# JuliaLinearAlgebra/AlgebraicMultigrid.jl

Measured on AMD Instinct MI355X. Metric: V-cycle unknowns/sec + fine-level SpMV GB/s (% HBM peak), 3-D Poisson 256^3, higher is better.
Workload: dtype f64

## Files before the change

### algebraicmultigrid.jl_amd/csrc/hip/amghip.hip

```cpp
#include "amghip_internal.hpp"
#include "gs_schedule.hpp"
#include "csr_ops.hpp"
#include "gmres_kernels.hpp"

namespace {

constexpr int64_t kGraphAutoRows = 65536;

struct Level {
  int64_t n = 0, nc = 0;
  amgh_csr A, S, P, R;
  bool has_S = false;
  amgh_smoother_t pre{}, post{};
  real *res = nullptr, *cx = nullptr, *cb = nullptr, *tmp = nullptr;
  real* il = nullptr;
  amgh_csr* smat() { return has_S ? &S : &A; }
  amgh_csr Pp, Rp;
  bool lo_ok = false;
  real* lo_val = nullptr;
  CodedCols lo_cc;
  bool r_stream = false, p_stream = false;
  bool lo_want = false;
  bool coarse_lo = false;
  bool nat_freed = false;
// ... 1323 lines not shown
}

static int ensure_pcg_bufs(amgh_t* h) {
  if (h->pc_r) return AMGH_OK;
  const int64_t n = fine_n(h);
  RC_TRY(dev_alloc(&h->pc_r, n));
  RC_TRY(dev_alloc(&h->pc_c, n));
  RC_TRY(dev_alloc(&h->pc_u, n));
  h->ws_bytes += 3 * kRealB * n;
  return AMGH_OK;
}

int amgh_solve_d(amgh_t* h, const real* b_d, real* x_d, int cycle_, int maxiter, double abstol, double reltol,
                 int calculate_residual, real* resid_hist, int* iters) {
  RC_TRY(check_ready(h));
  if (!b_d || !x_d || cycle_ < 0 || cycle_ > 2 || maxiter < 0) return AMGH_EINVAL;
  HIP_TRY(hipSetDevice(h->device));
  return solve_dev(h, b_d, x_d, cycle_, maxiter, abstol, reltol, calculate_residual, resid_hist, iters);
}

int amgh_solve(amgh_t* h, const real* b, real* x, int cycle_, int maxiter, double abstol, double reltol,
               int calculate_residual, real* resid_hist, int* iters) {
  RC_TRY(check_ready(h));
  if (!b || !x || cycle_ < 0 || cycle_ > 2 || maxiter < 0) return AMGH_EINVAL;
  HIP_TRY(hipSetDevice(h->device));
  const int64_t n = fine_n(h) * h->nrhs;
  HIP_TRY(hipMemcpyAsync(h->b0, b, sizeof(real) * n, hipMemcpyHostToDevice, h->stream));
  HIP_TRY(hipMemcpyAsync(h->x0, x, sizeof(real) * n, hipMemcpyHostToDevice, h->stream));
  RC_TRY(solve_dev(h, h->b0, h->x0, cycle_, maxiter, abstol, reltol, calculate_residual, resid_hist, iters));
  HIP_TRY(hipMemcpy(x, h->x0, sizeof(real) * n, hipMemcpyDeviceToHost));
  return AMGH_OK;
}

int amgh_precond_apply_d(amgh_t* h, const real* r_d, real* z_d, int cycle_) {
  RC_TRY(check_ready(h));
  if (!r_d || !z_d || cycle_ < 0 || cycle_ > 2) return AMGH_EINVAL;
  HIP_TRY(hipSetDevice(h->device));
  RC_TRY(bw_err_check());
  RC_TRY(vec_fill(h, z_d, fine_n(h) * h->nrhs, 0.0));
  return apply_cycle(h, z_d, r_d, cycle_, true);
}

int amgh_precond_apply(amgh_t* h, const real* r, real* z, int cycle_) {
  RC_TRY(check_ready(h));
  if (!r || !z) return AMGH_EINVAL;
  HIP_TRY(hipSetDevice(h->device));
  const int64_t n = fine_n(h) * h->nrhs;
  HIP_TRY(hipMemcpyAsync(h->b0, r, sizeof(real) * n, hipMemcpyHostToDevice, h->stream));
  RC_TRY(amgh_precond_apply_d(h, h->b0, h->x0, cycle_));
  HIP_TRY(hipStreamSynchronize(h->stream));
  RC_TRY(prof_flush(h));
  RC_TRY(bw_err_check());
  HIP_TRY(hipMemcpy(z, h->x0, sizeof(real) * n, hipMemcpyDeviceToHost));
  return AMGH_OK;
}

int amgh_cycle_d(amgh_t* h, int level, real* x_d, const real* b_d, int cycle_) {
  RC_TRY(check_ready(h));
  if (!x_d || !b_d || cycle_ < 0 || cycle_ > 2 || level < 0 || level > (int)h->levels.size()) return AMGH_EINVAL;
  HIP_TRY(hipSetDevice(h->device));
  if (level == (int)h->levels.size()) return coarse_solve(h, x_d, b_d);
  return cycle(h, level, x_d, b_d, cycle_, false);
}

int amgh_set_stream(amgh_t* h, void* stream) {
  if (!h) return AMGH_EINVAL;
  h->ext_stream = true;
  h->own_stream = h->own_stream ? h->own_stream : h->stream;
  h->stream = (hipStream_t)stream;
  return AMGH_OK;
}

// ... 654 lines not shown
  else if (!strcmp(name, "gs_nnz_per_wg")) g_gs_nnz_per_wg = value;
  else if (!strcmp(name, "gs_threads")) g_gs_threads = value;
  else if (!strcmp(name, "gs_block_inverse")) g_gs_block_inverse = value;
  else if (!strcmp(name, "gs_slots")) g_gs_slots = value;
  else if (!strcmp(name, "gs_xcd_map")) g_gs_xcd_map = value;
  else if (!strcmp(name, "gs_lpr")) g_gs_lpr = value;
  else if (!strcmp(name, "gs_il")) g_gs_il = value;
  else if (!strcmp(name, "trim_coded")) g_trim_coded = value;
  else if (!strcmp(name, "gs_wave_quad")) g_gs_wave_quad = value;
  else if (!strcmp(name, "pcg_fused")) g_pcg_fused = value;
  else if (!strcmp(name, "gs_tri_rb")) g_gs_tri_rb = value;
  else if (!strcmp(name, "gs_tri_rb1")) g_gs_tri_rb1 = value;
  else if (!strcmp(name, "gs_dti_pre")) g_gs_dti_pre = value;
  else if (!strcmp(name, "stream_xcd")) g_stream_xcd = value;
  else if (!strcmp(name, "tail_dense_rows")) g_tail_dense_rows = value < 0 ? 0 : value;
  else if (!strcmp(name, "tail_dense")) { g_tail_dense = value; g_sched_epoch++; }
  else if (!strcmp(name, "tail_dense_batch")) g_tail_dense_batch = value;
  else if (!strcmp(name, "gs_lean")) g_gs_lean = value;
  else if (!strcmp(name, "gs_sell")) g_gs_sell = value;
  else if (!strcmp(name, "gs_sample")) g_gs_sample = value;
  else if (!strcmp(name, "gs_tiny")) g_gs_tiny = value;
  else if (!strcmp(name, "gs_bw")) g_gs_bw = value;
  else if (!strcmp(name, "gs_bw_rows")) g_gs_bw_rows = value;
  else if (!strcmp(name, "gs_bw_chain")) g_gs_bw_chain = value;
  else if (!strcmp(name, "gs_bw_flow")) g_gs_bw_flow = value;
  else if (!strcmp(name, "gs_bw_spin")) g_gs_bw_spin = value;
  else if (!strcmp(name, "gs_bw_nc")) g_gs_bw_nc = value;
  else if (!strcmp(name, "gs_bw_nrhs")) g_gs_bw_nrhs = value;
  else if (!strcmp(name, "gs_bw_skip_pub")) g_gs_bw_skip_pub = value;
  else if (!strcmp(name, "gs_bw_min_rows")) g_gs_bw_min_rows = value;
  else if (!strcmp(name, "gs_bw_two_min_rows")) g_gs_bw_two_min_rows = value;
  else if (!strcmp(name, "gs_dup_launch")) g_gs_dup_launch = value < 0 ? 0 : value > 16 ? 16 : value;
  else if (!strcmp(name, "gs_flow_xzero")) g_gs_flow_xzero = value;
  else if (!strcmp(name, "gs_bw_grid")) g_gs_bw_grid = value < 0 ? 0 : value;
  else if (!strcmp(name, "gs_bw_grid_long")) g_gs_bw_grid_long = value < 0 ? 0 : value;
  else if (!strcmp(name, "gs_bw_dict")) g_gs_bw_dict = value != 0;
  else if (!strcmp(name, "gs_bw_inorder")) g_gs_bw_inorder = value != 0;
  else if (!strcmp(name, "stream_code")) g_stream_code = value != 0;
  else if (!strcmp(name, "gs_bw_relay")) g_gs_bw_relay = value == 0 ? 0 : BW_RELAY_W;
  else if (!strcmp(name, "rhs_il")) g_rhs_il = value;
  else if (!strcmp(name, "jacobi_zero")) g_jacobi_zero = value;
  else if (!strcmp(name, "gs_ept")) g_gs_ept = value;
  else if (!strcmp(name, "gs_merge")) g_gs_merge = value;
  else if (!strcmp(name, "gs_merge_force")) g_gs_merge_force = value;
  else if (!strcmp(name, "gs_merge_force_maxn")) g_gs_merge_force_maxn = value;
  else if (!strcmp(name, "gs_zone")) g_gs_zone = value;
  else if (!strcmp(name, "gs_coarse_lo")) g_gs_coarse_lo = value;
  else if (!strcmp(name, "gs_dense_tri")) g_gs_dense_tri = value;
  else if (!strcmp(name, "gs_dense_blk")) g_gs_dense_blk = value;
  else if (!strcmp(name, "gs_zone_t0_ns")) g_gs_zone_t0_ns = value;
  else if (!strcmp(name, "gs_zone_floor_ns")) g_gs_zone_floor_ns = value;
  else if (!strcmp(name, "gs_bigslot")) g_gs_bigslot = value;
  else if (!strcmp(name, "gs_flip")) g_gs_flip = value;
  else if (!strcmp(name, "gs_keep_lo")) g_gs_keep_lo = value;
  else if (!strcmp(name, "gs_super")) g_gs_super = value;
  else if (!strcmp(name, "gs_block_pipe")) g_gs_block_pipe = value;
  else return AMGH_EINVAL;
  ++g_sched_epoch;
  return AMGH_OK;
}

int amgh_debug_chain_timing(int enable, unsigned long long* out8) {
  if (enable && !g_chain_tim) {
    HIP_TRY(hipMalloc((void**)&g_chain_tim, 8 * sizeof(unsigned long long)));
    HIP_TRY(hipMemset(g_chain_tim, 0, 8 * sizeof(unsigned long long)));
  }
// ... 37 lines not shown
```

### algebraicmultigrid.jl_amd/csrc/hip/amghip_internal.hpp

```cpp
#pragma once
#include "amghip_kernels.hpp"
#include "gs_blocks.hpp"
#include "gs_flow.hpp"

#include <algorithm>
#include <chrono>
#include <cmath>
#include <cstdio>
#include <cstring>
#include <atomic>
#include <mutex>
#include <string>
#include <system_error>
#include <thread>
#include <utility>
#include <vector>

#include "../../../include/amghip.h"

using namespace amgh;

#define HIP_TRY(expr)                                   \
  do {                                                  \
    hipError_t e_ = (expr);                             \
// ... 323 lines not shown
int g_gs_block_pipe = 1;
int g_gs_super = 8;
int g_gs_coarse_lo = 1;
int g_gs_keep_lo = 1;
int g_gs_flip = 1;
int g_gs_bigslot = 1;
int g_gs_merge = 16;
int g_gs_zone_t0_ns = 3000;
int g_gs_zone_floor_ns = 0;
int g_gs_zone = 1;
int g_gs_merge_force_maxn = 0;
int g_gs_merge_force = 0;
int g_gs_xcd_map = 1;
int g_gs_slots = 1;
int g_jacobi_zero = 1;
int g_rhs_il = 1;
int g_gs_tiny = 1;
int g_gs_wave_quad = 1;
int g_gs_bw = 1;
int g_gs_bw_rows = 512;
int g_gs_bw_flow = 1;
int g_gs_bw_spin = 0;
int g_gs_bw_skip_pub = -1;
int g_gs_bw_nc = -1;
int g_gs_bw_nrhs = 1;
int g_gs_bw_chain = 1;
int g_stream_code = 1;
int g_trim_coded = 1;
int g_gs_bw_inorder = 0;
int g_gs_bw_dict = 1;
int g_gs_bw_relay = 3;
int g_gs_bw_grid = 0;
int g_gs_bw_grid_long = 512;
int g_gs_flow_xzero = 1;
int g_gs_dup_launch = 0;
int g_gs_bw_two_min_rows = 200000;
int g_gs_bw_min_rows = 30000;
int g_gs_sample = 1;
int g_gs_sell = 1;
int g_gs_lean = -1;
int g_gs_ept = 0;
int g_gs_lpr = 0;
int g_gs_il = 1;
int g_pcg_fused = 1;
int g_tail_dense_rows = 6144;
int g_tail_dense = 1;
int g_tail_dense_batch = 64;
int g_stream_xcd = 1;
int g_gs_dti_pre = 8;
int g_gs_tri_rb1 = 0;
int g_gs_tri_rb = 1;
int g_gs_dense_blk = 4096;
int g_gs_dense_tri = 1;
int g_gs_block_inverse = 1;

std::atomic<unsigned long long> g_sched_epoch{0};

unsigned long long* g_chain_tim = nullptr;

constexpr int kChainWidth = 1024;

__global__ void find_diag_kernel(const int32_t* rowptr, const int32_t* col, const real* val, int n,
                                 int32_t* dpos, real* diag) {
  const int i = blockIdx.x * blockDim.x + threadIdx.x;
  if (i >= n) return;
  int dp = -1;
// ... 54 lines not shown
```

### algebraicmultigrid.jl_amd/csrc/hip/csr_ops.hpp

```cpp
#pragma once
#include <atomic>

namespace {


template <int MODE, class CFG = DefaultCfg, bool CODED = false>
int launch_stream(const StreamArgs& a0, hipStream_t st, int ncolv = 1) {
  const int nrows = a0.row_end - a0.row_begin;
  if (nrows <= 0) return AMGH_OK;
  StreamArgs a = a0;
  a.ncolv = ncolv;
  const int nb = (nrows + CFG::ROWS - 1) / CFG::ROWS;
  const int64_t grid = (CFG::XCD || ncolv > 1) ? (int64_t)((nb + kNumXcd - 1) / kNumXcd) * kNumXcd * ncolv : nb;
  hipLaunchKernelGGL((csr_stream_kernel<MODE, CFG, CODED>), dim3((unsigned)grid), dim3(CFG::THREADS), 0, st, a);
  HIP_TRY(hipGetLastError());
  return AMGH_OK;
}

template <int MODE>
int launch_gs_level(const StreamArgs& a, int rows, hipStream_t st, int ncolv = 1) {
  const int width = a.row_end - a.row_begin;
  const int avg16 = std::max(16, rows);
  rows = 256;
  while (rows > g_gs_min_rows && (int64_t)rows * avg16 > (int64_t)g_gs_nnz_per_wg * 16) rows >>= 1;
// ... 547 lines not shown
  if (g_gs_merge > 1 && !sor && (backward ? g->mb : g->mf)) {
    lay = backward ? g->mb : g->mf;
    tri = backward ? &g->tri_b : &g->tri_f;
    s_key = 1.0;
    both_dirs = g->mf && g->mb;
  } else if (g_gs_merge > 1 && sor) {
    GsSchedule::SorSet* ss = sor_children(g, omega);
    if (ss && (ss->f || ss->b) && g->xstride == g->ncols && first && !x_resident) {
      HIP_TRY(hipStreamSynchronize(st));
      RC_TRY(gs_grow_xp_for_merged(g, &op->bytes));
    }
    if (ss && (backward ? ss->b : ss->f) && g->xstride > g->ncols) {
      lay = backward ? ss->b : ss->f;
      tri = backward ? &ss->tb : &ss->tf;
      s_key = omega;
      flip_scale = 2.0 - omega;
      both_dirs = ss->f && ss->b;
      sor = false;
    }
  }
  const int64_t xs = g->xstride;
  const bool il = g_gs_il && g_gs_lpr != 1 && lay != g && !g->bw.on && (ncolv == 8 || ncolv == 4 || ncolv == 2);
  if (first || !il) g->xil_cols = 0;
  bool il_s_ok = false;
  if (il && g->xil_cap < xs * ncolv) {
    HIP_TRY(hipStreamSynchronize(st));
    ++g_sched_epoch;
    hipFree(g->xil); g->xil = nullptr; g->xil_cap = 0;
    RC_TRY(dev_alloc(&g->xil, xs * ncolv));
    g->xil_cap = xs * ncolv;
    g->bytes += (int64_t)sizeof(real) * xs * ncolv; op->bytes += (int64_t)sizeof(real) * xs * ncolv;
    g->xil_cols = 0;
  }
  if (first) {
    if (!(reuse_b && g->bp_cols == ncolv))
      hipLaunchKernelGGL(gather_perm_kernel, dim3(grid_for(g->n), ncolv), dim3(256), 0, st, b, g->perm, g->bp, (int)g->n,
                         (int64_t)g->n, (int64_t)g->n);
    g->bp_cols = ncolv;
    if (x_resident) {
    } else if (xzero) {
      const bool flow_zero = g_gs_flow_xzero && g->bw.on && g->bw.flow.on && (g_gs_bw_flow || !g->bw.rec) && g->ncols == g->n && lay == g;
      if (!flow_zero) {
        const int64_t cnt = xs * ncolv;
        hipLaunchKernelGGL(fill_kernel, dim3(grid_for(cnt)), dim3(256), 0, st, g->xp, cnt, 0.0);
        if (il) {
          const int64_t ci = g->ncols * ncolv;
          hipLaunchKernelGGL(fill_kernel, dim3(grid_for(ci)), dim3(256), 0, st, g->xil, ci, 0.0);
          g->xil_cols = ncolv;
        }
      }
    } else {
      hipLaunchKernelGGL(gather_perm_kernel, dim3(grid_for(g->ncols), ncolv), dim3(256), 0, st, (const real*)x, g->permx,
                         g->xp, (int)g->ncols, (int64_t)g->ncols, xs);
    }
    HIP_TRY(hipGetLastError());
  }
  real* xp = g->xp;
  const real* rhs = g->bp;
  int64_t ldb = g->n;
  if (first) g->s_dir = -1;
  if (lay != g) {
    const bool flip = g->ncols == g->n && g->diag_nonzero && both_dirs && g_gs_flip &&
                      g->s_dir == (backward ? 0 : 1) && g->s_key == s_key;
    if (flip) {
      if (il) {
        real* sil = g->xil + g->ncols * ncolv;
#define AMGH_FLIP_IL(BS_) hipLaunchKernelGGL((gs_flip_rhs_il_kernel<BS_>), dim3(grid_for(g->n)), dim3(256), 0, st, (const real*)g->bp, \
                         (const real*)lay->diag, (const real*)xp, xp + g->ncols, (int)g->n, (int64_t)g->n, xs, flip_scale, sil)
// ... 30 lines not shown
      ra.row_begin = 0; ra.row_end = (int32_t)g->n;
      ra.ldx = xs; ra.ldy = xs; ra.ldb = g->n;
      RC_TRY(launch_stream<M_RESID>(ra, st, ncolv));
    }
    g->s_dir = backward ? 1 : 0;
    g->s_key = s_key;
    rhs = xp + g->ncols;
    ldb = xs;
  } else {
    g->s_dir = -1;
  }
  if (op->pipe_epoch && !(g->bw.on && g->bw.flow.on && (g_gs_bw_flow || !g->bw.rec))) return AMGH_ESTATE;
  if (g->bw.on) {
    hipError_t e = hipSuccess;
    const bool flow = g->bw.flow.on && (g_gs_bw_flow || !g->bw.rec);
    if (flow) {
      bw::FlowArgs<real> fa{g->bw.blocks, g->bw.flow.fd, g->bw.flow.srec, g->bw.flow.aux, g->bw.ext_col, g->bw.flow.fl_mb, g->bw.flow.fl_slot,
                            g->bw.flow.mbox, rhs, xp, omega, g->bw.head + 1, g->bw.nblocks, (int32_t)g->bw.flow.nmail,
                            g->bw.err, nullptr, (unsigned)g_gs_bw_spin, (int32_t)g_gs_bw_skip_pub};
      fa.ldb = ldb; fa.ldx = xs; fa.mail_stride = g->bw.flow.mail_stride;
      fa.xzero = (g_gs_flow_xzero && first && xzero && !x_resident && g->ncols == g->n) ? 1 : 0;
      if (ncolv > g->bw.flow.mcols) return AMGH_ESTATE;
      const bool dict = g->bw.flow.dict_on && (g_gs_bw_dict || !g->bw.flow.srec);
      if (op->pipe_epoch) {
        if (ncolv != 1 || !g->bw.flow.xon) return AMGH_ESTATE;
        fa.aux = g->bw.flow.xaux; fa.fl_mb = g->bw.flow.xfl_mb; fa.fl_slot = g->bw.flow.xfl_slot; fa.xlist = g->bw.flow.xlist;
        fa.epoch = op->pipe_epoch; fa.rmbox = op->pipe_rmbox; fa.grid = op->pipe_grid;
        if (dict) { fa.crec = g->bw.flow.crec; fa.dict = g->bw.flow.dict; fa.dict_ent = g->bw.flow.dict_ent; }
        e = bw::sweep_relay<real>(fa, g->bw.maxk, dict ? g->bw.flow.dict_lds : g->bw.flow.lds_max, sor, backward, st, BW_RELAY_W);
      } else if (ncolv == 1 && g_gs_bw_relay > 0) {
        fa.grid = g->bw.maxk > 6 ? (dict ? 0 : g_gs_bw_grid_long) : g_gs_bw_grid;
        fa.late = (g->bw.flow.late_ok && !g_gs_bw_inorder) ? 1 : 0;
        if (dict) { fa.crec = g->bw.flow.crec; fa.dict = g->bw.flow.dict; fa.dict_ent = g->bw.flow.dict_ent; }
        e = bw::sweep_relay<real>(fa, g->bw.maxk, dict ? g->bw.flow.dict_lds : g->bw.flow.lds_max, sor, backward, st, BW_RELAY_W);
      } else {
        if (dict) {
          fa.crec = g->bw.flow.crec; fa.dict = g->bw.flow.dict; fa.dict_ent = g->bw.flow.dict_ent;
          fa.dict_lds = (int32_t)(g->bw.flow.dict_lds - g->bw.flow.lds_max);
        }
        e = bw::sweep_flow<real>(fa, g->bw.maxk, g->bw.flow.lds_max, sor, backward, st, ncolv, g_gs_bw_nc >= 0 ? g_gs_bw_nc : (fa.crec ? 3 : 2));
      }
    } else {
      bw::Args<real> ba{g->bw.blocks, g->bw.rec, g->bw.ext_col, rhs, xp, ldb, xs, omega, 0, nullptr};
      if (g_gs_bw_chain && ncolv == 1 && g->bw.flags) {
        bw::ChainArgs<real> ca{ba, backward ? g->bw.sdep_ptr : g->bw.dep_ptr, backward ? g->bw.sdep : g->bw.dep, g->bw.flags, g->bw.head,
                               g->bw.nblocks, g->bw.err};
        e = bw::sweep_chain<real>(ca, g->bw.maxk, g->bw.lds_max, sor, backward, st);
      } else {
        e = bw::sweep<real>(ba, g->bw.maxk, g->bw.launch_ptr, g->bw.lds_max, sor, backward, ncolv, st);
      }
    }
    if (e != hipSuccess) return -(1000 + (int)e);
  }
  if (il) {
    if (g->xil_cols != ncolv) RC_TRY(il_copy_rows(ncolv, xp, xs, g->xil, 0, il_s_ok ? g->ncols : xs, st));
    else if (!il_s_ok) RC_TRY(il_copy_rows(ncolv, xp, xs, g->xil, g->ncols, g->n, st));
    g->xil_cols = ncolv;
  }
  const int ns = (int)lay->segs.size();
  for (int kk = 0; kk < ns * (1 + g_gs_dup_launch); ++kk) {
    const int k = kk / (1 + g_gs_dup_launch);
    const GsSchedule::Seg& s = lay->segs[backward ? ns - 1 - k : k];
    if (s.chain) {
      ChainArgs c{};
      c.col = lay->col; c.val = lay->val; c.x = xp; c.bp = rhs; c.diag = lay->diag;
      c.rowmeta = lay->rowmeta; c.desc = lay->desc; c.omega = omega; c.tim = g_chain_tim;
// ... 61 lines not shown
        SlotIlArgs ia{};
        ia.wcol = sa.wcol; ia.wval = sa.wval; ia.slot_row = sa.slot_row; ia.wmeta = sa.wmeta; ia.diag = sa.diag;
        ia.xil = g->xil; ia.x = xp; ia.omega = omega; ia.slot0 = s.slot0; ia.nslots = s.nslots;
        ia.xcd_map = (g_gs_xcd_map && s.nslots >= 768) ? 1 : 0;
        ia.soff = (int32_t)g->ncols; ia.ldx = xs;
        const int grid = ia.xcd_map ? ((s.nslots + kNumXcd - 1) / kNumXcd) * kNumXcd : s.nslots;
        RC_TRY(launch_slot_il(ia, sor, ncolv, grid, st));
        HIP_TRY(hipGetLastError());
        continue;
      }
      const int ncv = (ncolv % 8 == 0) ? 8 : (ncolv % 4 == 0) ? 4 : (ncolv % 2 == 0) ? 2 : 1;
      sa.ncolv = ncolv / ncv;
      const int grid = ((xmap || sa.ncolv > 1) ? ((s.nslots + kNumXcd - 1) / kNumXcd) * kNumXcd : s.nslots) * sa.ncolv;
      int lpr = 1;
      if (lay != g && ncolv == 1 && g_gs_lpr != 1) {
        const int avg = s.rows / 16;
        lpr = g_gs_lpr > 1 ? g_gs_lpr : (avg >= 56 ? 16 : avg >= 48 ? 8 : 1);
      }
      int ept = 1;
      if (lay != g && ncolv == 1) ept = g_gs_ept > 0 ? g_gs_ept : ((s.nslots > 1024 && lpr == 1 && s.rows / 16 < 16) ? 2 : 1);
      if (lpr > 1 || ept > 1) { RC_TRY(launch_slot_lpr(sa, sor, lpr, ept, grid, st)); HIP_TRY(hipGetLastError()); continue; }
      RC_TRY(launch_slot(sa, sor, ncv, grid, st));
      HIP_TRY(hipGetLastError());
    } else {
      StreamArgs a{};
      a.rowptr = lay->rowptr; a.col = lay->col; a.val = lay->val;
      a.x = xp; a.y = xp; a.b = rhs; a.dpos = lay->dpos; a.diag = lay->diag; a.perm = nullptr; a.omega = omega;
      a.row_begin = lay->lvl_ptr[s.l0]; a.row_end = lay->lvl_ptr[s.l0 + 1];
      a.ldx = xs; a.ldy = xs; a.ldb = ldb;
      RC_TRY(sor ? launch_gs_level<M_SOR>(a, s.rows, st, ncolv) : launch_gs_level<M_GS>(a, s.rows, st, ncolv));
      if (il) RC_TRY(il_copy_rows(ncolv, xp, xs, g->xil, a.row_begin, a.row_end - a.row_begin, st));
    }
  }
  if (last && !no_scatter) {
    hipLaunchKernelGGL(scatter_perm_kernel, dim3(grid_for(g->n), ncolv), dim3(256), 0, st, (const real*)xp, g->perm, x,
                       (int)g->n, xs, (int64_t)g->n);
    HIP_TRY(hipGetLastError());
  }
  return AMGH_OK;
}

}
```

### algebraicmultigrid.jl_amd/csrc/hip/gs_flow.hpp

```cpp
#pragma once
#include "gs_blocks.hpp"

namespace amgh {
namespace bw {

constexpr int32_t kPubFwd = 1 << 30;
constexpr int32_t kPubBwd = (int32_t)(1u << 31);
constexpr int32_t kPubMask = (1 << 30) - 1;
#ifndef BW_FLOW_WAVES
#define BW_FLOW_WAVES 4
#endif
#ifndef BW_FLOW_DEPTH
#define BW_FLOW_DEPTH 4
#endif

struct FlowDesc {
  int32_t aux;
  int32_t npost;
  int32_t pad0, pad1;
};
constexpr int kStepRowBits = 11, kStepCntBits = 7, kStepNeedMax = (1 << 14) - 1;
inline uint32_t step_word(int r0, int nr, int need) { return (uint32_t)r0 | ((uint32_t)nr << kStepRowBits) | ((uint32_t)need << (kStepRowBits + kStepCntBits)); }

constexpr int32_t kRemoteCell = (int32_t)(1u << 31);
// ... 341 lines not shown
    }
  }
  return true;
}

typedef unsigned int u32x4 __attribute__((ext_vector_type(4)));
typedef unsigned int u32x2 __attribute__((ext_vector_type(2)));

template <typename R>
struct FlowArgs {
  const Desc* blocks; const FlowDesc* fd;
  const unsigned char* srec; const uint32_t* aux;
  const int32_t* ext_col; const int32_t* fl_mb; const uint16_t* fl_slot;
  void* mbox;
  const R* b; R* x; R omega;
  unsigned long long* head;
  int32_t nblocks;
  int32_t nmail;
  int32_t* err;
  long long* tim;
  unsigned int spin_limit;
  int32_t skip_pub;
  int64_t ldb = 0, ldx = 0, mail_stride = 0;
  int32_t lds_stride = 0;
  int32_t ncols = 1, ngroups = 1;
  int32_t xzero = 0;
  uint32_t epoch = 0;
  const unsigned char* crec = nullptr; const unsigned char* dict = nullptr; const int32_t* dict_ent = nullptr;
  int32_t dict_lds = 0;
  const int32_t* xlist = nullptr;
  const void* rmbox = nullptr;
  int32_t late = 0;
  int32_t grid = 0;
};

template <typename R> struct Mail;
template <> struct Mail<double> {
  static constexpr int kBytes = 16;
  typedef u32x4 cell;
  static __device__ __forceinline__ cell load(__amdgpu_buffer_rsrc_t rs, unsigned off) { return __builtin_amdgcn_raw_buffer_load_b128(rs, off, 0, 16); }
  static __device__ __forceinline__ cell load_sys(__amdgpu_buffer_rsrc_t rs, unsigned off) { return __builtin_amdgcn_raw_buffer_load_b128(rs, off, 0, 17); }
  static __device__ __forceinline__ void store(__amdgpu_buffer_rsrc_t rs, unsigned off, double v, unsigned epoch) {
    const unsigned long long u = (unsigned long long)__double_as_longlong(v);
    cell c; c.x = (unsigned)u; c.y = epoch; c.z = (unsigned)(u >> 32); c.w = epoch;
    __builtin_amdgcn_raw_buffer_store_b128(c, rs, off, 0, 16);
  }
  static __device__ __forceinline__ bool valid(const cell& c, unsigned epoch) { return c.y == epoch && c.w == epoch; }
  static __device__ __forceinline__ double value(const cell& c) { return __longlong_as_double((long long)(((unsigned long long)c.z << 32) | c.x)); }
};
template <> struct Mail<float> {
  static constexpr int kBytes = 8;
  typedef u32x2 cell;
  static __device__ __forceinline__ cell load(__amdgpu_buffer_rsrc_t rs, unsigned off) { return __builtin_amdgcn_raw_buffer_load_b64(rs, off, 0, 16); }
  static __device__ __forceinline__ cell load_sys(__amdgpu_buffer_rsrc_t rs, unsigned off) { return __builtin_amdgcn_raw_buffer_load_b64(rs, off, 0, 17); }
  static __device__ __forceinline__ void store(__amdgpu_buffer_rsrc_t rs, unsigned off, float v, unsigned epoch) {
    cell c; c.x = __float_as_uint(v); c.y = epoch;
    __builtin_amdgcn_raw_buffer_store_b64(c, rs, off, 0, 16);
  }
  static __device__ __forceinline__ bool valid(const cell& c, unsigned epoch) { return c.y == epoch; }
  static __device__ __forceinline__ float value(const cell& c) { return __uint_as_float(c.x); }
};

typedef unsigned int u32x3 __attribute__((ext_vector_type(3)));
typedef int i32x4 __attribute__((ext_vector_type(4)));
template <int NDW> struct Dw;
template <> struct Dw<1> { typedef unsigned int type; };
// ... 515 lines not shown
```

### algebraicmultigrid.jl_amd/csrc/hip/gs_relay.hpp

```cpp
#pragma once
#include "gs_flow.hpp"

namespace amgh {
namespace bw {

#ifndef BW_RELAY_W
#define BW_RELAY_W 3
#endif

#ifndef BW_RELAY_SPIN
#define BW_RELAY_SPIN 48u
#endif
#ifndef BW_RELAY_DEPTH_SHORT
#define BW_RELAY_DEPTH_SHORT 3
#endif
#ifndef BW_RELAY_DEPTH_LONG
#define BW_RELAY_DEPTH_LONG 2
#endif
template <int MAXK> struct RelayDepth { static constexpr int value = MAXK <= 12 ? BW_RELAY_DEPTH_SHORT : BW_RELAY_DEPTH_LONG; };
#ifndef BW_RELAY_FETCH_SLEEP
#define BW_RELAY_FETCH_SLEEP 4
#endif
#ifndef BW_RELAY_FETCH_PD
#define BW_RELAY_FETCH_PD 1
// ... 28 lines not shown
  const int ns = d.nlev;
  const int nxb = (int)(((size_t)(d.nrows + d.next + 1) * sizeof(R) + 15) & ~(size_t)15);
  const unsigned spin_limit = a.spin_limit ? a.spin_limit : (1u << 22);
  unsigned char* lds = lds_all;
  R* xl = (R*)lds;
  unsigned int* ctl = (unsigned int*)(lds + nxb);
  R* x = a.x;
  if (fetcher) {
    constexpr int EU = 4;
    const R* xc = uniform_ptr(x);
    const int nfar = BWD ? d.npre + (d.next - d.npre - f.npost) : d.next - d.npre;
    if (a.xzero) {
      for (int e0 = 0; e0 < d.next; e0 += 64) { const int i = e0 + lane; if (i < d.next) xl[d.nrows + i] = (R)0; }
    } else
    for (int e0 = 0; e0 < nfar; e0 += 64 * EU) {
      int32_t ec[EU]; int es[EU];
#pragma unroll
      for (int k = 0; k < EU; ++k) {
        const int i = e0 + lane + 64 * k;
        es[k] = BWD ? (i < d.npre ? i : i + f.npost) : d.npre + i;
        ec[k] = a.ext_col[i < nfar ? d.ext0 + es[k] : 0];
      }
#pragma unroll
      for (int k = 0; k < EU; ++k) pin(ec[k]);
      R xe[EU];
#pragma unroll
      for (int k = 0; k < EU; ++k) xe[k] = xc[ec[k]];
#pragma unroll
      for (int k = 0; k < EU; ++k) pin(xe[k]);
#pragma unroll
      for (int k = 0; k < EU; ++k) { const int i = e0 + lane + 64 * k; if (i < nfar) xl[d.nrows + es[k]] = xe[k]; }
    }
    if (lane == 0) { xl[d.nrows + d.next] = (R)0; ctl[0] = 0u; ctl[1] = 0u; ctl[2] = 0u; ctl[3] = 0u; }
    fetcher_barrier();
#ifdef BW_RELAY_FETCH_PRIO
    __builtin_amdgcn_s_setprio(BW_RELAY_FETCH_PRIO);
#endif
    constexpr int U = 3;
    int nf = BWD ? f.npost : d.npre;
    int f0 = d.ext0 + (BWD ? d.npre : 0);
    if (a.xlist) {
      const int l0 = a.xlist[4 * (int64_t)ob], lf = a.xlist[4 * (int64_t)ob + 1], lb = a.xlist[4 * (int64_t)ob + 2];
      nf = __builtin_amdgcn_readfirstlane(BWD ? lb : lf);
      f0 = __builtin_amdgcn_readfirstlane(BWD ? l0 + lf : l0);
    }
    const __amdgpu_buffer_rsrc_t rs_mail = __builtin_amdgcn_make_buffer_rsrc(uniform_ptr(a.mbox), 0, 0x7ffffff0, 0x00020000);
    const __amdgpu_buffer_rsrc_t rs_rmail = __builtin_amdgcn_make_buffer_rsrc(uniform_ptr(const_cast<void*>(a.rmbox ? a.rmbox : (const void*)a.mbox)), 0, 0x7ffffff0, 0x00020000);
    unsigned total_spins = 0;
    bool fail = false;
#ifdef BW_RELAY_STAMPS
    long long* t_seen = a.tim + 4 * (int64_t)a.nblocks + 384 * (int64_t)a.nblocks + ((int64_t)a.nmail + 1024);
    long long poll_sum = 0, poll_max = 0, npoll = 0;
#endif
#if BW_RELAY_FETCH_PD > 1 && !defined(BW_RELAY_STAMPS)
    constexpr int PD = BW_RELAY_FETCH_PD;
    for (int w0 = 0; w0 < nf && !fail; w0 += 64 * U) {
      int32_t mb[U]; int slot[U]; bool ok[U];
#pragma unroll
      for (int u = 0; u < U; ++u) {
        const int e = w0 + 64 * u + lane;
        mb[u] = a.fl_mb[e < nf ? f0 + e : f0];
        slot[u] = a.fl_slot[e < nf ? f0 + e : f0];
        ok[u] = !(e < nf);
      }
      int first = 0;
      typename M::cell q[PD][U];
// ... 125 lines not shown
      asm_load<O::CTAIL + 1>(o.ct, voff, rs_rec, s0 + (unsigned)(O::NCC - 1) * sd);
    } else {
#pragma unroll
      for (int c = 0; c < O::NVC - 1; ++c) asm_load<4>(o.vf[c], voff, rs_rec, s0 + (unsigned)c * sd);
      asm_load<O::VTAIL>(o.vt, voff, rs_rec, s0 + (unsigned)(O::NVC - 1) * sd);
#pragma unroll
      for (int c = 0; c < O::NCC - 1; ++c) asm_load<4>(o.cf[c], voff, rs_rec, s0 + (unsigned)(O::NVC + c) * sd);
      asm_load<O::CTAIL + 1>(o.ct, voff, rs_rec, s0 + (unsigned)(O::NVC + O::NCC - 1) * sd);
    }
    asm_load<RB / 4>(o.bb, (unsigned)tt * RB, rs_b, (unsigned)r0 * RB);
  };
  O ops[D];
  {
    constexpr int XW = W >= 4 ? 2 : 4;
    if (a.xzero) {
      for (int p = wv * 64 + lane; p < d.nrows; p += 64 * W) xl[p] = (R)0;
    } else
    for (int p0 = wv * 64 * XW; p0 < d.nrows; p0 += 64 * XW * W) {
      R xv[XW];
#pragma unroll
      for (int k = 0; k < XW; ++k) { const int p = p0 + lane + 64 * k; xv[k] = x[d.row0 + (p < d.nrows ? p : 0)]; }
#pragma unroll
      for (int k = 0; k < XW; ++k) pin(xv[k]);
#pragma unroll
      for (int k = 0; k < XW; ++k) { const int p = p0 + lane + 64 * k; if (p < d.nrows) xl[p] = xv[k]; }
    }
    if constexpr (DICT) {
      const int32_t de = a.dict_ent[ob];
      const int nchunk = (((unsigned)de >> 24) + 1) * NVC;
      const u32x4* dg = (const u32x4*)(a.dict + (size_t)(de & 0xffffff) * 16);
      u32x4* dl = (u32x4*)(lds + nxb + 16);
      for (int i = wv * 64 + lane; i < nchunk; i += 64 * W) dl[i] = dg[i];
    }
    asm volatile("s_waitcnt vmcnt(0)" ::: "memory");
#pragma unroll
    for (int j = 0; j < D; ++j) issue(ops[j], wv + j * W);
  }
  __syncthreads();
  __builtin_amdgcn_s_setprio(2);
  const long long t_loaded = a.tim ? wall_clock64() : 0;
  const int32_t pubdir = BWD ? kPubBwd : kPubFwd;
  const bool mute = a.skip_pub == tk;
  const unsigned spare = (unsigned)a.nmail + (unsigned)(ob & 1023);
  bool gave_up = false, bail = false;
  const unsigned xl_base = (unsigned)__builtin_amdgcn_readfirstlane((int)lds_addr(xl));
  const unsigned ctl_off = xl_base + (unsigned)nxb;
  const unsigned dict_base = ctl_off + 16u;
#ifdef BW_RELAY_STAMPS
  const unsigned stamp_base = xl_base + (unsigned)nxb + 16u;
  i32x4 rs_pub = make_rsrc(a.tim + 4 * (int64_t)a.nblocks + 384 * (int64_t)a.nblocks);
  if (!a.tim) rs_pub.z = 0;
#endif
  auto step = [&](const O& o, int kk) {
#ifdef BW_RELAY_STAMPS
    const long long t_rec = wall_clock64();
#endif
    constexpr bool PRE = MAXK <= 18;
    constexpr int NOFF = (PRE && !LATE) ? MAXK : 1;
    auto col_addr = [&](int k) {
      const u32x4 cw = o.cchunk(k >> 3);
      const unsigned w = ((k >> 1) & 3) == 0 ? cw.x : ((k >> 1) & 3) == 1 ? cw.y : ((k >> 1) & 3) == 2 ? cw.z : cw.w;
      return xl_base + ((k & 1) ? (w >> 16) : (w & 0xffffu));
    };
    unsigned off[NOFF];
#pragma unroll
    for (int k = 0; k < NOFF; ++k) off[k] = col_addr(k);
    const int32_t pw = o.pub();
// ... 176 lines not shown
#endif
  };
#ifdef BW_RELAY_STAMPS
  constexpr int L = O::NLOAD, S = 3;
#else
  constexpr int L = O::NLOAD, S = 2;
#endif
  const int nsw = ns > wv ? (ns - wv + W - 1) / W : 0;
  int k = 0;
  if (nsw >= D) {
#pragma unroll
    for (int j = 0; j < D; ++j) {
      if (j == 0) flow_wait<(D - 1) * L>(ops[0]);
      else if (j == 1) flow_wait<(D - 2) * L + 1 * (L + S)>(ops[1 < D ? 1 : 0]);
      else if (j == 2) flow_wait<(D > 2 ? D - 3 : 0) * L + 2 * (L + S)>(ops[2 < D ? 2 : 0]);
      else flow_wait<(D > 3 ? D - 4 : 0) * L + 3 * (L + S)>(ops[3 < D ? 3 : 0]);
      step(ops[j], wv + j * W);
      issue(ops[j], wv + (j + D) * W);
    }
    for (k = D; k + D <= nsw; k += D) {
#pragma unroll
      for (int j = 0; j < D; ++j) {
        flow_wait<(D - 1) * (L + S)>(ops[j]);
        step(ops[j], wv + (k + j) * W);
        issue(ops[j], wv + (k + j + D) * W);
      }
    }
  }
  asm volatile("s_waitcnt vmcnt(0)" ::: "memory");
#pragma unroll
  for (int j = 0; j < D - 1; ++j)
    if (k + j < nsw) { flow_wait<0>(ops[j]); step(ops[j], wv + (k + j) * W); }
  if (gave_up && lane == 0) *a.err = 2;
#ifdef BW_RELAY_STAMPS
  if (a.tim) {
    asm volatile("s_waitcnt lgkmcnt(0)" ::: "memory");
    for (int kk = wv; kk < ns && kk < 128; kk += W)
      if (lane < 3) a.tim[4 * (int64_t)a.nblocks + 384 * (int64_t)ob + 3 * kk + lane] = lds_get<long long>(stamp_base + 24u * (unsigned)kk + 8u * (unsigned)lane);
  }
#endif
  if (a.tim && lane == 0) {
    long long* tt = a.tim + 4 * (int64_t)ob;
    if (wv == 0) {
      tt[0] = t_start; tt[1] = t_loaded;
      unsigned xcc = 0;
#ifdef BW_RELAY_STAMPS
      asm volatile("s_getreg_b32 %0, hwreg(HW_REG_XCC_ID)" : "=s"(xcc));
#endif
      tt[3] = (long long)(xcc & 15u);
    }
    if (wv == (ns - 1) % W) tt[2] = wall_clock64();
  }
}

template <typename R, bool SOR, bool BWD, int MAXK, int W, bool DICT = false, bool LATE = false>
__global__ __launch_bounds__(64 * (W + 1), DICT ? RelayWavesD<MAXK>::value : RelayWaves<MAXK>::value) void gs_bw_relay_kernel(FlowArgs<R> a) {
  extern __shared__ __attribute__((aligned(16))) unsigned char lds_all[];
  static_assert(W >= 2 && W <= 7, "walker waves per block");
  const int wv = __builtin_amdgcn_readfirstlane((int)(threadIdx.x >> 6));
  const int lane = (int)(threadIdx.x & 63u);
  const unsigned int units = (unsigned int)a.nblocks;
  const bool persistent = gridDim.x < units;
  const unsigned int draws = units + (persistent ? gridDim.x : 0u);
  unsigned long long* s_ticket = (unsigned long long*)lds_all;
  if (blockIdx.x < 2048u) for (unsigned i = 0; i < (blockIdx.x >> 5); ++i) __builtin_amdgcn_s_sleep(14);
  for (;;) {
// ... 107 lines not shown
```

Baseline: 1.191 billion.

## Fold permutation gather/scatter into relay GS sweep and skip fine x zero-fill

```diff
diff --git a/algebraicmultigrid.jl_amd/csrc/hip/amghip.hip b/algebraicmultigrid.jl_amd/csrc/hip/amghip.hip
--- a/algebraicmultigrid.jl_amd/csrc/hip/amghip.hip
+++ b/algebraicmultigrid.jl_amd/csrc/hip/amghip.hip
@@ -1379,12 +1379,21 @@
   return AMGH_OK;
 }
 
+bool fine_x_write_only(const amgh_t* h, int cyc) {
+  if (!g_gs_bw_fold || h->levels.empty() || tail_here(h, 0, cyc)) return false;
+  Level* L = h->levels[0];
+  const GsSchedule* g = L->smat()->gs;
+  const bool lo = L->lo_ok && (g_gs_keep_lo || L->nat_freed) && g && g->nblk == 0;
+  auto gs = [](const amgh_smoother_t& s) { return (s.kind == AMGH_SMOOTH_GS || s.kind == AMGH_SMOOTH_SOR) && s.iter > 0; };
+  return lo && g->n == L->n && !(g->dti_f && g_gs_dense_tri && g_gs_block_inverse) && gs(L->pre) && gs(L->post);
+}
+
 int amgh_precond_apply_d(amgh_t* h, const real* r_d, real* z_d, int cycle_) {
   RC_TRY(check_ready(h));
   if (!r_d || !z_d || cycle_ < 0 || cycle_ > 2) return AMGH_EINVAL;
   HIP_TRY(hipSetDevice(h->device));
   RC_TRY(bw_err_check());
-  RC_TRY(vec_fill(h, z_d, fine_n(h) * h->nrhs, 0.0));
+  if (!fine_x_write_only(h, cycle_)) RC_TRY(vec_fill(h, z_d, fine_n(h) * h->nrhs, 0.0));
   return apply_cycle(h, z_d, r_d, cycle_, true);
 }
 
@@ -2105,6 +2114,7 @@
   else if (!strcmp(name, "gs_bw_two_min_rows")) g_gs_bw_two_min_rows = value;
   else if (!strcmp(name, "gs_dup_launch")) g_gs_dup_launch = value < 0 ? 0 : value > 16 ? 16 : value;
   else if (!strcmp(name, "gs_flow_xzero")) g_gs_flow_xzero = value;
+  else if (!strcmp(name, "gs_bw_fold")) g_gs_bw_fold = value != 0;
   else if (!strcmp(name, "gs_bw_grid")) g_gs_bw_grid = value < 0 ? 0 : value;
   else if (!strcmp(name, "gs_bw_grid_long")) g_gs_bw_grid_long = value < 0 ? 0 : value;
   else if (!strcmp(name, "gs_bw_dict")) g_gs_bw_dict = value != 0;
diff --git a/algebraicmultigrid.jl_amd/csrc/hip/amghip_internal.hpp b/algebraicmultigrid.jl_amd/csrc/hip/amghip_internal.hpp
--- a/algebraicmultigrid.jl_amd/csrc/hip/amghip_internal.hpp
+++ b/algebraicmultigrid.jl_amd/csrc/hip/amghip_internal.hpp
@@ -379,6 +379,7 @@
 int g_gs_bw_relay = 3;
 int g_gs_bw_grid = 0;
 int g_gs_bw_grid_long = 512;
+int g_gs_bw_fold = 1;
 int g_gs_flow_xzero = 1;
 int g_gs_dup_launch = 0;
 int g_gs_bw_two_min_rows = 200000;
diff --git a/algebraicmultigrid.jl_amd/csrc/hip/csr_ops.hpp b/algebraicmultigrid.jl_amd/csrc/hip/csr_ops.hpp
--- a/algebraicmultigrid.jl_amd/csrc/hip/csr_ops.hpp
+++ b/algebraicmultigrid.jl_amd/csrc/hip/csr_ops.hpp
@@ -603,8 +603,12 @@
     g->bytes += (int64_t)sizeof(real) * xs * ncolv; op->bytes += (int64_t)sizeof(real) * xs * ncolv;
     g->xil_cols = 0;
   }
+  const bool relay1 = g_gs_bw_fold && ncolv == 1 && g->bw.on && g->bw.flow.on && (g_gs_bw_flow || !g->bw.rec) && g_gs_bw_relay > 0 &&
+                      !op->pipe_epoch && lay == g && g->bw.flow.dict_on && (g_gs_bw_dict || !g->bw.flow.srec);
+  const bool fold_b = relay1 && first && !(reuse_b && g->bp_cols == ncolv);
+  const bool fold_x = relay1 && last && !no_scatter;
   if (first) {
-    if (!(reuse_b && g->bp_cols == ncolv))
+    if (!(reuse_b && g->bp_cols == ncolv) && !fold_b)
       hipLaunchKernelGGL(gather_perm_kernel, dim3(grid_for(g->n), ncolv), dim3(256), 0, st, b, g->perm, g->bp, (int)g->n,
                          (int64_t)g->n, (int64_t)g->n);
     g->bp_cols = ncolv;
@@ -701,6 +705,9 @@
         fa.grid = g->bw.maxk > 6 ? (dict ? 0 : g_gs_bw_grid_long) : g_gs_bw_grid;
         fa.late = (g->bw.flow.late_ok && !g_gs_bw_inorder) ? 1 : 0;
         if (dict) { fa.crec = g->bw.flow.crec; fa.dict = g->bw.flow.dict; fa.dict_ent = g->bw.flow.dict_ent; }
+        if (fold_b || fold_x) fa.perm = g->perm;
+        if (fold_b) fa.b_nat = b;
+        if (fold_x) fa.x_nat = x;
         e = bw::sweep_relay<real>(fa, g->bw.maxk, dict ? g->bw.flow.dict_lds : g->bw.flow.lds_max, sor, backward, st, BW_RELAY_W);
       } else {
         if (dict) {
@@ -828,7 +835,7 @@
       if (il) RC_TRY(il_copy_rows(ncolv, xp, xs, g->xil, a.row_begin, a.row_end - a.row_begin, st));
     }
   }
-  if (last && !no_scatter) {
+  if (last && !no_scatter && !fold_x) {
     hipLaunchKernelGGL(scatter_perm_kernel, dim3(grid_for(g->n), ncolv), dim3(256), 0, st, (const real*)xp, g->perm, x,
                        (int)g->n, xs, (int64_t)g->n);
     HIP_TRY(hipGetLastError());
diff --git a/algebraicmultigrid.jl_amd/csrc/hip/gs_flow.hpp b/algebraicmultigrid.jl_amd/csrc/hip/gs_flow.hpp
--- a/algebraicmultigrid.jl_amd/csrc/hip/gs_flow.hpp
+++ b/algebraicmultigrid.jl_amd/csrc/hip/gs_flow.hpp
@@ -397,6 +397,7 @@
   const void* rmbox = nullptr;
   int32_t late = 0;
   int32_t grid = 0;
+  const int32_t* perm = nullptr; const R* b_nat = nullptr; R* x_nat = nullptr;
 };
 
 template <typename R> struct Mail;
diff --git a/algebraicmultigrid.jl_amd/csrc/hip/gs_relay.hpp b/algebraicmultigrid.jl_amd/csrc/hip/gs_relay.hpp
--- a/algebraicmultigrid.jl_amd/csrc/hip/gs_relay.hpp
+++ b/algebraicmultigrid.jl_amd/csrc/hip/gs_relay.hpp
@@ -84,6 +84,7 @@
       for (int k = 0; k < EU; ++k) { const int i = e0 + lane + 64 * k; if (i < nfar) xl[d.nrows + es[k]] = xe[k]; }
     }
     if (lane == 0) { xl[d.nrows + d.next] = (R)0; ctl[0] = 0u; ctl[1] = 0u; ctl[2] = 0u; ctl[3] = 0u; }
+    if constexpr (DICT) if (a.b_nat) __syncthreads();
     fetcher_barrier();
 #ifdef BW_RELAY_FETCH_PRIO
     __builtin_amdgcn_s_setprio(BW_RELAY_FETCH_PRIO);
@@ -275,7 +276,26 @@
       u32x4* dl = (u32x4*)(lds + nxb + 16);
       for (int i = wv * 64 + lane; i < nchunk; i += 64 * W) dl[i] = dg[i];
     }
+    if (DICT && a.b_nat) {
+      R* bo = const_cast<R*>(a.b) + d.row0;
+      const int32_t* pm = a.perm + d.row0;
+      for (int p0 = wv * 64 * XW; p0 < d.nrows; p0 += 64 * XW * W) {
+        int32_t pi[XW];
+#pragma unroll
+        for (int k = 0; k < XW; ++k) { const int p = p0 + lane + 64 * k; pi[k] = pm[p < d.nrows ? p : 0]; }
+#pragma unroll
+        for (int k = 0; k < XW; ++k) pin(pi[k]);
+        R bv[XW];
+#pragma unroll
+        for (int k = 0; k < XW; ++k) bv[k] = a.b_nat[pi[k]];
+#pragma unroll
+        for (int k = 0; k < XW; ++k) pin(bv[k]);
+#pragma unroll
+        for (int k = 0; k < XW; ++k) { const int p = p0 + lane + 64 * k; if (p < d.nrows) bo[p] = bv[k]; }
+      }
+    }
     asm volatile("s_waitcnt vmcnt(0)" ::: "memory");
+    if constexpr (DICT) if (a.b_nat) __syncthreads();
 #pragma unroll
     for (int j = 0; j < D; ++j) issue(ops[j], wv + j * W);
   }
@@ -518,6 +538,27 @@
   for (int j = 0; j < D - 1; ++j)
     if (k + j < nsw) { flow_wait<0>(ops[j]); step(ops[j], wv + (k + j) * W); }
   if (gave_up && lane == 0) *a.err = 2;
+  if (DICT && a.x_nat) {
+    const unsigned* ctlw = (const unsigned*)(lds + nxb);
+    for (;;) {
+      const unsigned bl = __hip_atomic_load(ctlw + 2, __ATOMIC_RELAXED, __HIP_MEMORY_SCOPE_WORKGROUP);
+      const unsigned dn = __hip_atomic_load(ctlw + 1, __ATOMIC_ACQUIRE, __HIP_MEMORY_SCOPE_WORKGROUP);
+      if (bl != 0u) { bail = true; break; }
+      if (dn >= (unsigned)ns) break;
+      __builtin_amdgcn_s_sleep(1);
+    }
+    if (!bail) {
+      constexpr int XW = W >= 4 ? 2 : 4;
+      const int32_t* pm = a.perm + d.row0;
+      for (int p0 = wv * 64 * XW; p0 < d.nrows; p0 += 64 * XW * W) {
+        int32_t pi[XW];
+#pragma unroll
+        for (int k = 0; k < XW; ++k) { const int p = p0 + lane + 64 * k; pi[k] = pm[p < d.nrows ? p : 0]; }
+#pragma unroll
+        for (int k = 0; k < XW; ++k) { const int p = p0 + lane + 64 * k; if (p < d.nrows) a.x_nat[pi[k]] = xl[p]; }
+      }
+    }
+  }
 #ifdef BW_RELAY_STAMPS
   if (a.tim) {
     asm volatile("s_waitcnt lgkmcnt(0)" ::: "memory");
```

After: 1.213 billion (median of 6 runs). 1.9% higher.
